# luigifreda/pyslam

Measured on AMD Instinct MI355X. Metric: RGB-D frames/sec fused (640x480, 5 mm voxel TSDF), higher is better.
Workload: dtype f32; 1 GPU; synthetic_640x480_5mm: synthetic 640x480 RGB-D @ 30 Hz stream, 5 mm TSDF (sdf_trunc 0.04 m, depth_trunc 4 m), 64 posed frames per step resident in HBM, Open3D ScalableTSDFVolume semantics; mode=multi-frame sweep (hv_tsdf_integrate_batch), units_allocated=31946, parity_pinned=False, clock_ramp_steps=60, full=False, build_digest=135281701958bda57bf956d25b5e2e59f6e6b8a8ce9266cc3e6c719ccc494ef5

## Files before the change

pyslam_amd/csrc/hv_tsdf.hip:

```cpp
#include <algorithm>
#include <array>
#include <cmath>
#include <cstring>
#include <numeric>

#include "hv_tsdf_device.h"

__global__ __launch_bounds__(256) void k_tsdf_multiplier_table(HvFrameParams P, float *__restrict__ out) {
    const int i = blockIdx.x * blockDim.x + threadIdx.x;
    if (i >= P.H * P.W) return;
    out[i] = hv_multiplier(P, i % P.W, i / P.W);
}


__global__ __launch_bounds__(256) void k_tsdf_prep_touch(HvTable table, int32_t *__restrict__ stamp,
                                                          int32_t *__restrict__ list, int parity,
                                                          const void *__restrict__ depth_raw,
                                                          const uint8_t *__restrict__ rgb,
                                                          uint2 *__restrict__ frame_px, HvFrameParams P,
                                                          int n_touch_blocks) {
    const int64_t npx = (int64_t)P.H * P.W;
    if ((int)blockIdx.x >= n_touch_blocks) {
        const int64_t i = (int64_t)((int)blockIdx.x - n_touch_blocks) * blockDim.x + threadIdx.x;
        if (i >= npx) return;
// ... 69 lines not shown

template <int ZB>
__device__ __forceinline__ void hv_tsdf_slabs(const HvFrameParams &P, const uint2 *__restrict__ frame_px, char *__restrict__ unit, int wordb,
                                              float (&pc)[4][3], float inc0, float inc1, float inc2) {
    float tv[ZB][4];
    uint32_t cv[ZB][4];
    unsigned mask = 0;
    bool near_plane = false;
#pragma unroll
    for (int c = 0; c < 4; ++c) {
        const float e = pc[c][2] + (float)ZB * inc2;
        near_plane |= (int)(fminf(pc[c][2], e) < 0x1p-10f) & (int)(fmaxf(pc[c][2], e) > -0x1p-10f);
    }
    if (P.tiled || __any(near_plane)) {
#pragma unroll
        for (int zz = 0; zz < ZB; ++zz) {
#pragma unroll
            for (int c = 0; c < 4; ++c) {
                if (hv_tsdf_eval_fast<true, false>(P, frame_px, nullptr, pc[c][0], pc[c][1], pc[c][2], tv[zz][c], cv[zz][c]))
                    mask |= 1u << (zz * 4 + c);
                pc[c][0] += inc0;
                pc[c][1] += inc1;
                pc[c][2] += inc2;
            }
        }
    } else {
#pragma unroll
        for (int zz = 0; zz < ZB; ++zz) {
#pragma unroll
            for (int c = 0; c < 4; ++c) {
                if (hv_tsdf_eval_fast<false, false>(P, frame_px, nullptr, pc[c][0], pc[c][1], pc[c][2], tv[zz][c], cv[zz][c]))
                    mask |= 1u << (zz * 4 + c);
                pc[c][0] += inc0;
                pc[c][1] += inc1;
                pc[c][2] += inc2;
            }
        }
    }
    float4 vt[ZB];
    uint4 vw[ZB], vr[ZB], vg[ZB], vb[ZB];
#pragma unroll
    for (int zz = 0; zz < ZB; ++zz) {
        if ((mask >> (zz * 4)) & 15u) {
            const int q = (wordb + zz * HV_TSDF_RR) >> 2;
            vt[zz] = ((const float4 *)(unit + 0 * HV_TSDF_PLANE_BYTES))[q];
            vw[zz] = ((const uint4 *)(unit + 1 * HV_TSDF_PLANE_BYTES))[q];
            vr[zz] = ((const uint4 *)(unit + 2 * HV_TSDF_PLANE_BYTES))[q];
            vg[zz] = ((const uint4 *)(unit + 3 * HV_TSDF_PLANE_BYTES))[q];
            vb[zz] = ((const uint4 *)(unit + 4 * HV_TSDF_PLANE_BYTES))[q];
        }
    }
#pragma unroll
    for (int zz = 0; zz < ZB; ++zz) {
        const unsigned m = (mask >> (zz * 4)) & 15u;
        if (m) {
            hv_tsdf_apply(m & 1u, tv[zz][0], cv[zz][0], vt[zz].x, vw[zz].x, vr[zz].x, vg[zz].x, vb[zz].x);
            hv_tsdf_apply(m & 2u, tv[zz][1], cv[zz][1], vt[zz].y, vw[zz].y, vr[zz].y, vg[zz].y, vb[zz].y);
            hv_tsdf_apply(m & 4u, tv[zz][2], cv[zz][2], vt[zz].z, vw[zz].z, vr[zz].z, vg[zz].z, vb[zz].z);
            hv_tsdf_apply(m & 8u, tv[zz][3], cv[zz][3], vt[zz].w, vw[zz].w, vr[zz].w, vg[zz].w, vb[zz].w);
            const int q = (wordb + zz * HV_TSDF_RR) >> 2;
            ((float4 *)(unit + 0 * HV_TSDF_PLANE_BYTES))[q] = vt[zz];
            ((uint4 *)(unit + 1 * HV_TSDF_PLANE_BYTES))[q] = vw[zz];
            ((uint4 *)(unit + 2 * HV_TSDF_PLANE_BYTES))[q] = vr[zz];
            ((uint4 *)(unit + 3 * HV_TSDF_PLANE_BYTES))[q] = vg[zz];
            ((uint4 *)(unit + 4 * HV_TSDF_PLANE_BYTES))[q] = vb[zz];
        }
    }
}

__global__ __launch_bounds__(256) void k_tsdf_integrate(HvTable table, const int32_t *__restrict__ list,
                                                         int parity, char *__restrict__ pool,
                                                         const uint2 *__restrict__ frame_px, HvFrameParams P,
                                                         HvStatus *status, int32_t status_seq) {
    int n_touched = table.counters[HV_CNT_TOUCH(parity)];
    if (n_touched > table.max_blocks) n_touched = table.max_blocks;
    if (blockIdx.x == 0 && threadIdx.x == 0) {
        table.counters[HV_CNT_TOUCH(parity ^ 1)] = 0;
        hv_publish_status(table, status, status_seq);
    }
    const int wave = threadIdx.x >> 6;
    const int lane = threadIdx.x & 63;
    const int x = lane >> 2;
    const int y0 = (lane & 3) << 2;
    const int z0 = wave * 4;
    const float inc0 = P.ext_scaled_col2[0], inc1 = P.ext_scaled_col2[1], inc2 = P.ext_scaled_col2[2];

    for (int t = blockIdx.x; t < n_touched; t += gridDim.x) {
        const int32_t slot = list[t];
        const int32_t idx = table.vals[slot];
        if (idx < 0) continue;
        int32_t ux, uy, uz;
        hv_unpack_key(table.keys[slot], ux, uy, uz);
        const double o0 = (double)ux * P.unit_length;
        const double o1 = (double)uy * P.unit_length;
        const double o2 = (double)uz * P.unit_length;
        const float p0 = (float)((double)(P.half_voxel_length_f + P.voxel_length_f * (float)x) + o0);
        const float p2 = (float)((double)P.half_voxel_length_f + o2);
        float pc[4][3];
#pragma unroll
        for (int c = 0; c < 4; ++c) {
            const float p1 = (float)((double)(P.half_voxel_length_f + P.voxel_length_f * (float)(y0 + c)) + o1);
#pragma unroll
            for (int r = 0; r < 3; ++r) {
                pc[c][r] = ((P.ext[r * 4 + 0] * p0 + P.ext[r * 4 + 1] * p1) + P.ext[r * 4 + 2] * p2) + P.ext[r * 4 + 3];
            }
        }
        for (int s = 0; s < z0; ++s) {
#pragma unroll
            for (int c = 0; c < 4; ++c) {
                pc[c][0] += inc0;
                pc[c][1] += inc1;
                pc[c][2] += inc2;
            }
        }
        char *unit = pool + (int64_t)idx * HV_TSDF_UNIT_BYTES;
        constexpr int ZB = 2;
#pragma unroll
        for (int zb = 0; zb < 4; zb += ZB) hv_tsdf_slabs<ZB>(P, frame_px, unit, hv_tsdf_word(x, y0, z0 + zb), pc, inc0, inc1, inc2);
    }
}

__device__ __forceinline__ void hv_touch_batch_patch(const HvTable &table, const HvFrameParams &P, const void *depth_f, const int patch,
                                                     HvTouchScratch &scratch, const int f, unsigned long long *__restrict__ frame_mask,
                                                     int32_t *__restrict__ stamp, int32_t *__restrict__ list, const int batch_stamp,
                                                     const int parity) {
    const unsigned long long fbit = 1ull << f;
    hv_touch_patch(table, P, depth_f, patch, scratch,
                   [&](unsigned long long key, int32_t ux, int32_t uy, int32_t uz) {
                       if (!hv_unit_hits_tile(P, ux, uy, uz)) return;
                       const int32_t slot = hv_table_insert(table, key);
                       if (slot < 0) return;
                       const unsigned long long seen = __hip_atomic_load(&frame_mask[slot], __ATOMIC_RELAXED, __HIP_MEMORY_SCOPE_AGENT);
                       const int32_t stamped = __hip_atomic_load(&stamp[slot], __ATOMIC_RELAXED, __HIP_MEMORY_SCOPE_AGENT);
                       if (!(seen & fbit)) atomicOr(&frame_mask[slot], fbit);
                       if (stamped != batch_stamp) {
                           const int32_t old = atomicExch(&stamp[slot], batch_stamp);
                           if (old != batch_stamp) {
                               const int32_t at = atomicAdd(&table.counters[HV_CNT_TOUCH(parity)], 1);
                               if (at < table.max_blocks) list[at] = slot;
                           }
                       }
                   });
}

__global__ __launch_bounds__(256) void k_tsdf_prep_touch_batch(HvTable table, int32_t *__restrict__ stamp,
                                                                unsigned long long *__restrict__ frame_mask,
                                                                int32_t *__restrict__ list, int batch_stamp,
                                                                const char *__restrict__ depth_raw, int64_t depth_stride,
                                                                const uint8_t *__restrict__ rgb,
                                                                uint2 *__restrict__ frame_px,
                                                                const HvFrameParams *__restrict__ Ps, int n_prep_blocks,
                                                                int n_touch_blocks, int n_frames, int parity,
                                                                const float *__restrict__ mult12) {
    int f, bx;
    const bool touch_role = (int)blockIdx.x < n_touch_blocks * n_frames;
    if (touch_role) {
        f = (int)blockIdx.x / n_touch_blocks;
        bx = (int)blockIdx.x % n_touch_blocks;
    } else {
        const int b = (int)blockIdx.x - n_touch_blocks * n_frames;
        f = b / n_prep_blocks;
        bx = b % n_prep_blocks;
    }
    const HvFrameParams &P = Ps[f];
    const int64_t npx = (int64_t)P.H * P.W;
    const void *depth_f = depth_raw + (int64_t)f * depth_stride;
    const uint8_t *rgb_f = rgb + (int64_t)f * npx * 3;
    if (!touch_role) {
        hv_pack_px4(P, f, ((int64_t)bx * blockDim.x + threadIdx.x) * 4, depth_f, rgb_f, frame_px, mult12);
        return;
    }
    __shared__ HvTouchScratch scratch[4];
    const int patch = bx * 4 + (int)(threadIdx.x / HV_WAVE);
    if (patch < hv_touch_patches(P))
        hv_touch_batch_patch(table, P, depth_f, patch, scratch[threadIdx.x / HV_WAVE], f, frame_mask, stamp, list, batch_stamp, parity);
}

typedef float hv_f2 __attribute__((ext_vector_type(2)));

__device__ __forceinline__ hv_f2 hv_fma2(hv_f2 a, hv_f2 b, hv_f2 c) { return __builtin_elementwise_fma(a, b, c); }
__device__ __forceinline__ hv_f2 hv_splat(float x) { return hv_f2{x, x}; }

struct HvSweepFrameK {
    hv_f2 e04, e15, e26, e37;
    float e8, e11;
    hv_f2 e9_10, i01;
    float i2;
};
__device__ __forceinline__ HvSweepFrameK hv_sweep_frame_k(const HvFrameParams *__restrict__ Ps, int f) {
    const float *k = Ps[f].sweep_k;
    return HvSweepFrameK{hv_f2{k[0], k[1]}, hv_f2{k[2], k[3]}, hv_f2{k[4], k[5]}, hv_f2{k[6], k[7]}, k[8], k[9], hv_f2{k[10], k[11]}, hv_f2{k[12], k[13]}, k[14]};
}

static constexpr unsigned HV_SWEEP_XCD_GROUP = 2;
__device__ __forceinline__ int hv_sweep_items(const int n_units, const int parts) {
    constexpr int G = HV_SWEEP_XCD_GROUP;
    return (n_units + 8 * G - 1) / (8 * G) * 8 * G * parts;
}
__device__ __forceinline__ void hv_sweep_item(const unsigned item, const unsigned parts, int &t, int &part) {
    constexpr unsigned G = HV_SWEEP_XCD_GROUP;
    const unsigned xcd = item & 7u, j = item >> 3;
    const unsigned g = j / (G * parts), within = j % (G * parts);
    t = (int)((g * 8 + xcd) * G + within / parts);
    part = (int)(within % parts);
}

static constexpr int HV_WAIT_VMCNT0 = 0x0f70;
struct HvPlaneWords {
    float vt;
    uint32_t vw, r, g, b;
};
template <int ZH, int ZB, bool TW, typename Updated, typename Finish>
__device__ __forceinline__ void hv_sweep_epilogue(char *__restrict__ unit, const int wordb, Updated updated, Finish finish) {
    constexpr int NP = ZH / ZB;
    static_assert(ZH % ZB == 0, "whole passes");
    auto load = [&](const int p, HvPlaneWords (&w)[ZB]) __attribute__((always_inline)) {
#pragma unroll
        for (int k = 0; k < ZB; ++k) {
            const int z = p * ZB + k;
            if (updated(z)) {
                const int q = wordb + z * HV_TSDF_RR;
                if (TW) {
                    w[k].vt = ((const float *)(unit + 0 * HV_TSDF_PLANE_BYTES))[q];
                    w[k].vw = ((const uint32_t *)(unit + 1 * HV_TSDF_PLANE_BYTES))[q];
                }
                w[k].r = ((const uint32_t *)(unit + 2 * HV_TSDF_PLANE_BYTES))[q];
                w[k].g = ((const uint32_t *)(unit + 3 * HV_TSDF_PLANE_BYTES))[q];
                w[k].b = ((const uint32_t *)(unit + 4 * HV_TSDF_PLANE_BYTES))[q];
            }
        }
    };
    auto store = [&](const int p, const HvPlaneWords (&w)[ZB]) __attribute__((always_inline)) {
#pragma unroll
        for (int k = 0; k < ZB; ++k) {
            const int z = p * ZB + k;
            if (updated(z)) {
                const int q = wordb + z * HV_TSDF_RR;
                HvPlaneWords o = w[k];
                finish(z, o);
                ((float *)(unit + 0 * HV_TSDF_PLANE_BYTES))[q] = o.vt;
                ((uint32_t *)(unit + 1 * HV_TSDF_PLANE_BYTES))[q] = o.vw;
                ((uint32_t *)(unit + 2 * HV_TSDF_PLANE_BYTES))[q] = o.r;
                ((uint32_t *)(unit + 3 * HV_TSDF_PLANE_BYTES))[q] = o.g;
                ((uint32_t *)(unit + 4 * HV_TSDF_PLANE_BYTES))[q] = o.b;
            }
        }
    };
#pragma unroll
    for (int p = 0; p < NP; ++p) {
        HvPlaneWords w[ZB];
        load(p, w);
        __builtin_amdgcn_sched_barrier(0);
        __builtin_amdgcn_s_waitcnt(HV_WAIT_VMCNT0);
        store(p, w);
        __builtin_amdgcn_sched_barrier(0);
    }
}

static constexpr int HV_SWEEP_ZH = 4;
static constexpr int HV_SWEEP_SPLIT = 8;
static constexpr int HV_SWEEP_WAVES = 64 / HV_SWEEP_ZH / HV_SWEEP_SPLIT;
static constexpr int HV_SWEEP_WPE = 4;
static_assert(HV_SWEEP_ZH % 2 == 0, "voxels are folded in pairs");

struct HvSweepGather {
    uint2 rec[HV_SWEEP_ZH];
    float mm[HV_SWEEP_ZH], zk[HV_SWEEP_ZH];
    bool ok[HV_SWEEP_ZH];
};

__global__ __launch_bounds__(64 * HV_SWEEP_WAVES, HV_SWEEP_WPE) void k_tsdf_sweep(
    HvTable table, const int32_t *__restrict__ list, const unsigned long long *__restrict__ frame_mask,
    char *__restrict__ pool, const uint2 *__restrict__ frame_px, const HvFrameParams *__restrict__ Ps, int n_frames,
    int general, const float *__restrict__ mult, int parity) {
    constexpr int ZH = HV_SWEEP_ZH, SPLIT = HV_SWEEP_SPLIT, WAVES = HV_SWEEP_WAVES;
    int n_units = table.counters[HV_CNT_TOUCH(parity)];
    if (n_units > table.max_blocks) n_units = table.max_blocks;
    const int wave = __builtin_amdgcn_readfirstlane(threadIdx.x >> 6);
    const int lane = threadIdx.x & 63;
    const HvFrameParams &P0 = Ps[0];
    const float vl = P0.voxel_length_f, hl = P0.half_voxel_length_f;
    const double unit_length = P0.unit_length;
    const bool tiled = P0.tiled != 0;
    const int npx = P0.H * P0.W;
    const hv_f2 F = {P0.fx, P0.fy}, C = {P0.cx, P0.cy};
    const uint32_t lo = __float_as_uint(0.0001f);
    const uint32_t wlim = __float_as_uint(P0.safe_width_f) - lo, hlim = __float_as_uint(P0.safe_height_f) - lo;
    const uint32_t W24 = (uint32_t)P0.W;
    const float ntrunc = -P0.sdf_trunc_f, tinv = P0.sdf_trunc_inv_f;
    const __amdgpu_buffer_rsrc_t rs_m = __builtin_amdgcn_make_buffer_rsrc((void *)mult, 0, npx * 4, 0x00020000);
    const int n_items = hv_sweep_items(n_units, SPLIT);
    for (int item = blockIdx.x; item < n_items; item += gridDim.x) {
        int t, part;
        hv_sweep_item(item, SPLIT, t, part);
        if (t >= n_units) continue;
        const int task = part * WAVES + wave;
        const int cg = task & 3;
        const int z0 = (task >> 2) * ZH;
        const int x = cg * 4 + (lane >> 4);
        const int y = lane & 15;
        const int32_t slot = list[t];
        const int32_t idx = table.vals[slot];
        unsigned long long mask = frame_mask[slot];
        if (idx < 0 || mask == 0ull) continue;
        int32_t ux, uy, uz;
        hv_unpack_key(table.keys[slot], ux, uy, uz);
        const double o0 = (double)ux * unit_length, o1 = (double)uy * unit_length, o2 = (double)uz * unit_length;
        bool near = false;
        if (lane < n_frames && ((mask >> lane) & 1ull)) {
            const HvFrameParams &Pl = Ps[lane];
            const float bx = (float)((double)(hl + vl * (float)(cg * 4)) + o0), by = (float)((double)hl + o1),
                        bz = (float)((double)(hl + vl * (float)z0) + o2);
            const float zmin = (Pl.ext[8] * bx + Pl.ext[9] * by + Pl.ext[10] * bz + Pl.ext[11]) + fminf(Pl.ext[8] * (3.0f * vl), 0.f) +
                               fminf(Pl.ext[9] * (15.0f * vl), 0.f) + fminf(Pl.ext[10] * ((float)(ZH - 1) * vl), 0.f);
            near = !(zmin > 0.03f);
        }
        const bool near_any = __any(near);
        char *unit = pool + (int64_t)idx * HV_TSDF_UNIT_BYTES;
        const int wordb = z0 * HV_TSDF_RR + cg * 64 + lane;
        float vt[ZH];
        uint32_t vw[ZH];
#pragma unroll
        for (int zz = 0; zz < ZH; ++zz) {
            const int q = wordb + zz * HV_TSDF_RR;
            vt[zz] = ((const float *)(unit + 0 * HV_TSDF_PLANE_BYTES))[q];
// ... 552 lines not shown
    for (int attempt = 0;; ++attempt) {
        tsdf_next_frame(v, P, parity);
        if (attempt > 0) HV_HIP(hipMemsetAsync(&v->table.counters[HV_CNT_TOUCH0], 0, HV_CNT_TOUCH_SPAN_BYTES, v->stream));
        rc = tsdf_launch_touch(v, v->stream, P, parity, d_depth, d_rgb);
        if (rc != HV_OK) return rc;
        if (!checked) break;
        rc = hv_claims_fit(v);
        if (rc == HV_OK) break;
        if (rc != HV_RETRY_CLAIM || attempt >= 8) return rc == HV_RETRY_CLAIM ? HV_ERR_CAPACITY : rc;
        make_frame_params(v, H, W, intr, T_cw, depth_scale, depth_trunc, depth_dtype, &P);
    }
    return tsdf_launch_integrate(v, P, parity);
}

int check_tsdf_args(hv_volume *v, const void *depth, const uint8_t *rgb, int H, int W,
                           const double *intr, const double *T_cw, int frames) {
    HV_REQUIRE(v != nullptr, HV_ERR_INVALID, "hv_tsdf_integrate: null volume");
    HV_REQUIRE(v->cfg.mode == HV_MODE_TSDF, HV_ERR_MODE, "hv_tsdf_integrate: volume is not in TSDF mode");
    HV_REQUIRE(depth != nullptr && rgb != nullptr && intr != nullptr && T_cw != nullptr, HV_ERR_INVALID,
               "[ScalableTSDFVolume::Integrate] Unsupported image format.");
    HV_REQUIRE(H > 0 && W > 0 && frames > 0, HV_ERR_INVALID, "hv_tsdf_integrate: empty image");
    HV_REQUIRE((int64_t)H * W <= v->cfg.max_points, HV_ERR_CAPACITY,
               "hv_tsdf_integrate: image %dx%d exceeds max_points=%lld", W, H, (long long)v->cfg.max_points);
    return HV_OK;
}

extern "C" {

int hv_tsdf_integrate(hv_volume *v, const void *depth, int32_t depth_dtype, const uint8_t *rgb,
                      int32_t height, int32_t width, const double *intr, const double *T_cw,
                      double depth_scale, double depth_trunc, int32_t loc) {
    int rc = check_tsdf_args(v, depth, rgb, height, width, intr, T_cw, 1);
    if (rc != HV_OK) return rc;
    HV_HIP(hipSetDevice(v->device));
    const size_t npx = (size_t)height * width;
    const void *d_depth = nullptr;
    const uint8_t *d_rgb = nullptr;
    rc = hv_stage_frame(v, depth, depth_dtype, rgb, npx, loc, &d_depth, &d_rgb);
    if (rc != HV_OK) return rc;
    return tsdf_integrate_one(v, d_depth, depth_dtype, d_rgb, height, width, intr, T_cw,
                              depth_scale, depth_trunc);
}

}

size_t tsdf_batch_scratch(size_t rec_bytes, size_t npx, int B, size_t *params_offset) {
    const size_t px_bytes = rec_bytes * npx * (size_t)B;
    *params_offset = (px_bytes + 255) & ~(size_t)255;
    return px_bytes + 256 + sizeof(HvFrameParams) * (size_t)B;
}

int tsdf_integrate_batch_impl(hv_volume *v, const void *depth, const void *const *depth_ptrs, int32_t depth_dtype,
                                     const uint8_t *rgb, const void *const *rgb_ptrs, int32_t n_frames, int32_t height,
                                     int32_t width, const double *intr, const double *T_cw, double depth_scale,
                                     double depth_trunc, int32_t loc) {
    int rc = HV_OK;
    HV_HIP(hipSetDevice(v->device));
    const size_t npx = (size_t)height * width;
    const size_t dsz = depth_dtype == HV_DEPTH_U16 ? 2 : 4;
    const void *d_depth = nullptr, *d_rgb = nullptr;
    int host_set = -1;
    if (loc == HV_HOST) {
        rc = hv_stage_frames(v, depth_ptrs, depth, npx * dsz, rgb_ptrs, rgb, npx * 3, n_frames, &d_depth, &d_rgb, &host_set);
        if (rc != HV_OK) return rc;
    } else {
        d_depth = depth;
        d_rgb = rgb;
    }
    if (n_frames == 1) {
        if (host_set >= 0) HV_HIP(hipStreamWaitEvent(v->stream, v->hs_dev_ready[host_set], 0));
        rc = tsdf_integrate_one(v, d_depth, depth_dtype, (const uint8_t *)d_rgb, height, width, intr, T_cw, depth_scale, depth_trunc);
        if (rc != HV_OK) return rc;
        if (host_set >= 0) return hv_stage_frames_consumed(v, host_set, v->stream);
        return HV_OK;
    }
    const bool pipeline_on = !(getenv("HV_TSDF_PIPELINE") && atoi(getenv("HV_TSDF_PIPELINE")) == 0);
    const int sweep_form = getenv("HV_TSDF_SWEEP") && atoi(getenv("HV_TSDF_SWEEP")) == 2 ? 2 : 4;
    const bool rec12 = sweep_form == 4;
    const size_t rec_bytes = rec12 ? 12 : 8;
    const int general = getenv("HV_TSDF_BATCH_GENERAL") ? atoi(getenv("HV_TSDF_BATCH_GENERAL")) : 0;
    const int zs = getenv("HV_TSDF_SWEEP_ZS") ? atoi(getenv("HV_TSDF_SWEEP_ZS")) : (v->owner_world >= 4 ? 2 : 1);
    const int sweep_grid = 65536;
    bool chain_ok = v->pipe_armed && v->pipe_version == v->content_version;
    v->content_version += 1;
    const int BMAX = HV_BATCH_MAX;
    for (int f0 = 0; f0 < n_frames; f0 += BMAX) {
        const int B = std::min(BMAX, n_frames - f0);
        bool checked = false;
        const int64_t max_before = v->cfg.max_blocks;
        rc = hv_capacity_gate(v, &checked);
        if (rc != HV_OK) return rc;
        if (v->cfg.max_blocks != max_before) chain_ok = false;
        const bool overlap = pipeline_on && chain_ok && !checked;
        if (v->stream_aux == nullptr) {
            HV_HIP(hipStreamCreateWithFlags(&v->stream_aux, hipStreamNonBlocking));
            HV_HIP(hipEventCreateWithFlags(&v->ev_prep, hipEventDisableTiming));
            HV_HIP(hipEventCreateWithFlags(&v->ev_presweep, hipEventDisableTiming));
        }
        hipStream_t ps = overlap ? v->stream_aux : v->stream;
        bool overlap_this = overlap;
        const int parity = v->batch_parity & 1;
        v->batch_parity = parity ^ 1;
        int32_t *d_list = v->touched_list + (size_t)parity * (size_t)v->cfg.max_blocks;
        unsigned long long *d_mask_rw = (unsigned long long *)v->touched_mask + (size_t)parity * (size_t)v->table_capacity;
        if (overlap) HV_HIP(hipStreamWaitEvent(v->stream_aux, v->ev_presweep, 0));
        if (host_set >= 0) HV_HIP(hipStreamWaitEvent(ps, v->hs_dev_ready[host_set], 0));
        const int ri = v->params_idx;
        v->params_idx = (ri + 1) & 3;
        if (v->pinned_params[ri] == nullptr) {
            HV_HIP(hipHostMalloc(&v->pinned_params[ri], sizeof(HvFrameParams) * BMAX));
            HV_HIP(hipEventCreateWithFlags(&v->params_ev[ri], hipEventDisableTiming));
        } else {
            HV_HIP(hipEventSynchronize(v->params_ev[ri]));
        }
        HvFrameParams *params = (HvFrameParams *)v->pinned_params[ri];
        for (int f = 0; f < B; ++f) {
            make_frame_params(v, height, width, intr, T_cw + 16 * (size_t)(f0 + f), depth_scale, depth_trunc, depth_dtype,
                              &params[f]);
            v->frame_counter += 1;
            params[f].frame_id = v->frame_counter;
        }
        int batch_stamp = v->frame_counter;
        v->last_touch_parity = parity;
        {
            const float *before = v->mult_table;
            const int mw = v->mult_W, mh = v->mult_H;
            float key_before[4];
            memcpy(key_before, v->mult_key, sizeof(key_before));
            rc = tsdf_multiplier_table(v, params[0]);
            if (rc != HV_OK) return rc;
            if (before != v->mult_table || mw != v->mult_W || mh != v->mult_H || memcmp(key_before, v->mult_key, sizeof(key_before)) != 0) {
                if (ps != v->stream) HV_HIP(hipStreamSynchronize(v->stream_aux));
                ps = v->stream;
                overlap_this = false;
                if (host_set >= 0) HV_HIP(hipStreamWaitEvent(ps, v->hs_dev_ready[host_set], 0));
            }
        }
        const float *d_mult = v->mult_table;
        size_t params_off = 0;
        const size_t want = tsdf_batch_scratch(rec_bytes, npx, B, &params_off);
        void **bb = parity ? &v->batch_buf2 : &v->batch_buf;
        size_t *bb_bytes = parity ? &v->batch_buf2_bytes : &v->batch_buf_bytes;
        if (*bb_bytes < want && v->stream_aux) HV_HIP(hipStreamSynchronize(v->stream_aux));
        rc = hv_ensure_buffer(v, bb, bb_bytes, want);
        if (rc != HV_OK) return rc;
        uint2 *d_px = (uint2 *)*bb;
        HvFrameParams *d_params = (HvFrameParams *)((char *)*bb + params_off);
        {
            const int n16 = (int)((sizeof(HvFrameParams) * (size_t)B + 15) / 16);
            hipLaunchKernelGGL(k_upload_words, dim3(1), dim3(256), 0, ps, (const uint4 *)params, (uint4 *)d_params, n16);
        }
        HV_HIP(hipEventRecord(v->params_ev[ri], ps));
        const int n_prep_blocks = (int)((npx + 1023) / 1024);
        const int n_touch_blocks = (hv_touch_patches(width, height, v->cfg.depth_sampling_stride) + 3) / 4;
        const void *c_depth = (const char *)d_depth + npx * dsz * (size_t)f0;
        const uint8_t *c_rgb = (const uint8_t *)d_rgb + npx * 3 * (size_t)f0;
        rc = tsdf_rectify(v, ps, &c_depth, depth_dtype, &c_rgb, B, height, width);
        if (rc != HV_OK) return rc;
        for (int attempt = 0;; ++attempt) {
            if (!v->touch_counters_clean) HV_HIP(hipMemsetAsync(&v->table.counters[HV_CNT_TOUCH0], 0, HV_CNT_TOUCH_SPAN_BYTES, v->stream));
            v->touch_counters_clean = true;
            hipLaunchKernelGGL(k_tsdf_prep_touch_batch, dim3((n_prep_blocks + n_touch_blocks) * B), dim3(256), 0, ps,
                               v->table, v->touched_stamp, d_mask_rw, d_list, batch_stamp,
                               (const char *)c_depth, (int64_t)(npx * dsz), c_rgb, d_px, (const HvFrameParams *)d_params, n_prep_blocks, n_touch_blocks, B, parity,
                               rec12 ? d_mult : (const float *)nullptr);
            if (!checked) break;
            rc = hv_claims_fit(v);
            if (rc == HV_OK) break;
            if (rc != HV_RETRY_CLAIM || attempt >= 8) return rc == HV_RETRY_CLAIM ? HV_ERR_CAPACITY : rc;
            v->frame_counter += 1;
            batch_stamp = v->frame_counter;
            v->touch_counters_clean = false;
            d_list = v->touched_list + (size_t)parity * (size_t)v->cfg.max_blocks;
            d_mask_rw = (unsigned long long *)v->touched_mask + (size_t)parity * (size_t)v->table_capacity;
        }
        HV_HIP(hipEventRecord(v->ev_presweep, v->stream));
        if (overlap_this) {
            HV_HIP(hipEventRecord(v->ev_prep, v->stream_aux));
            HV_HIP(hipStreamWaitEvent(v->stream, v->ev_prep, 0));
        }
        chain_ok = true;
        hv_profile_begin(v);
        const unsigned long long *d_mask = d_mask_rw;
        if (sweep_form == 2)
            hipLaunchKernelGGL(k_tsdf_sweep, dim3(sweep_grid), dim3(64 * HV_SWEEP_WAVES), 0, v->stream, v->table, (const int32_t *)d_list, d_mask,
                               (char *)v->pool, (const uint2 *)d_px, (const HvFrameParams *)d_params, B, general, d_mult, parity);
        else if (zs == 2)
            hipLaunchKernelGGL(k_tsdf_sweep_column<2>, dim3(sweep_grid), dim3(64), 0, v->stream, v->table, (const int32_t *)d_list, d_mask,
                               (char *)v->pool, (const uint2 *)d_px, (const HvFrameParams *)d_params, B, general, d_mult, parity);
        else
            hipLaunchKernelGGL(k_tsdf_sweep_column<1>, dim3(sweep_grid), dim3(64), 0, v->stream, v->table, (const int32_t *)d_list, d_mask,
                               (char *)v->pool, (const uint2 *)d_px, (const HvFrameParams *)d_params, B, general, d_mult, parity);
        hv_profile_end(v, B);
        hipLaunchKernelGGL(k_tsdf_batch_finish, dim3(1), dim3(1024), 0, v->stream, v->table, (const int32_t *)d_list, d_mask_rw, parity, v->d_status,
                           hv_next_status_seq(v));
        HV_HIP(hipGetLastError());
    }
    v->pipe_armed = true;
    v->pipe_version = v->content_version;
    if (host_set >= 0) return hv_stage_frames_consumed(v, host_set, v->stream);
    return HV_OK;
}

extern "C" {

int hv_tsdf_integrate_batch(hv_volume *v, const void *depth, int32_t depth_dtype, const uint8_t *rgb,
                            int32_t n_frames, int32_t height, int32_t width, const double *intr,
                            const double *T_cw, double depth_scale, double depth_trunc, int32_t loc) {
    int rc = check_tsdf_args(v, depth, rgb, height, width, intr, T_cw, n_frames);
    if (rc != HV_OK) return rc;
    return tsdf_integrate_batch_impl(v, depth, nullptr, depth_dtype, rgb, nullptr, n_frames, height, width, intr, T_cw, depth_scale,
                                     depth_trunc, loc);
}

int hv_tsdf_integrate_frames(hv_volume *v, const void *const *depth_frames, int32_t depth_dtype, const uint8_t *const *rgb_frames,
                             int32_t n_frames, int32_t height, int32_t width, const double *intr, const double *T_cw,
                             double depth_scale, double depth_trunc) {
    HV_REQUIRE(depth_frames != nullptr && rgb_frames != nullptr && n_frames >= 1, HV_ERR_INVALID, "hv_tsdf_integrate_frames: null argument");
    for (int f = 0; f < n_frames; ++f)
        HV_REQUIRE(depth_frames[f] != nullptr && rgb_frames[f] != nullptr, HV_ERR_INVALID, "hv_tsdf_integrate_frames: null frame %d", f);
    int rc = check_tsdf_args(v, depth_frames[0], rgb_frames[0], height, width, intr, T_cw, n_frames);
    if (rc != HV_OK) return rc;
    return tsdf_integrate_batch_impl(v, nullptr, depth_frames, depth_dtype, nullptr, (const void *const *)rgb_frames, n_frames, height,
                                     width, intr, T_cw, depth_scale, depth_trunc, HV_HOST);
}

int hv_tsdf_set_tile(hv_volume *v, int32_t u0, int32_t v0, int32_t u1, int32_t v1) {
    HV_REQUIRE(v != nullptr, HV_ERR_INVALID, "hv_tsdf_set_tile: null volume");
    HV_REQUIRE(v->cfg.mode == HV_MODE_TSDF, HV_ERR_MODE, "hv_tsdf_set_tile: volume is not in TSDF mode");
    HV_REQUIRE((u0 == 0 && v0 == 0 && u1 == 0 && v1 == 0) || (u0 >= 0 && v0 >= 0 && u1 > u0 && v1 > v0), HV_ERR_INVALID,
               "hv_tsdf_set_tile: empty tile");
    v->tile[0] = u0;
    v->tile[1] = v0;
    v->tile[2] = u1;
    v->tile[3] = v1;
    return HV_OK;
}

int hv_tsdf_set_color_order(hv_volume *v, int32_t bgr) {
    HV_REQUIRE(v != nullptr, HV_ERR_INVALID, "hv_tsdf_set_color_order: null volume");
    HV_REQUIRE(v->cfg.mode == HV_MODE_TSDF, HV_ERR_MODE, "hv_tsdf_set_color_order: volume is not in TSDF mode");
    v->color_bgr = bgr ? 1 : 0;
    return HV_OK;
}

int hv_tsdf_set_owner(hv_volume *v, int32_t rank, int32_t world_size) {
    HV_REQUIRE(v != nullptr, HV_ERR_INVALID, "hv_tsdf_set_owner: null volume");
    HV_REQUIRE(v->cfg.mode == HV_MODE_TSDF, HV_ERR_MODE, "hv_tsdf_set_owner: volume is not in TSDF mode");
    HV_REQUIRE(world_size >= 1 && rank >= 0 && rank < world_size, HV_ERR_INVALID, "hv_tsdf_set_owner: bad rank/world");
    v->owner_rank = rank;
    v->owner_world = world_size;
    return HV_OK;
}

int hv_tsdf_dump(hv_volume *v, int32_t *keys, float *tsdf, float *weight, double *color, int64_t *n_units) {
    HV_REQUIRE(v != nullptr && n_units != nullptr, HV_ERR_INVALID, "hv_tsdf_dump: null argument");
    HV_REQUIRE(v->cfg.mode == HV_MODE_TSDF, HV_ERR_MODE, "hv_tsdf_dump: volume is not in TSDF mode");
    int64_t nb = 0;
    int rc = hv_num_blocks(v, &nb);
    if (rc != HV_OK) return rc;
    *n_units = nb;
    if (nb == 0 || (keys == nullptr && tsdf == nullptr && weight == nullptr && color == nullptr)) return HV_OK;
    std::vector<int32_t> order, xyz;
    rc = hv_tsdf_key_order(v, nb, order, &xyz);
    if (rc != HV_OK) return rc;
    std::vector<char> unit((size_t)HV_TSDF_UNIT_BYTES);
    for (int64_t o = 0; o < nb; ++o) {
        const int64_t i = order[o];
        if (keys) memcpy(keys + o * 3, &xyz[o * 3], 12);
        if (!(tsdf || weight || color)) continue;
        HV_HIP(hipMemcpy(unit.data(), (char *)v->pool + i * unit.size(), unit.size(), hipMemcpyDeviceToHost));
        const float *pt = (const float *)unit.data();
        const uint32_t *pw = (const uint32_t *)(unit.data() + HV_TSDF_PLANE_BYTES);
        const uint32_t *pr = (const uint32_t *)(unit.data() + 2 * HV_TSDF_PLANE_BYTES);
        const uint32_t *pg = (const uint32_t *)(unit.data() + 3 * HV_TSDF_PLANE_BYTES);
        const uint32_t *pb = (const uint32_t *)(unit.data() + 4 * HV_TSDF_PLANE_BYTES);
        for (int x = 0; x < HV_TSDF_R; ++x)
            for (int y = 0; y < HV_TSDF_R; ++y)
                for (int z = 0; z < HV_TSDF_R; ++z) {
                    const int src = hv_tsdf_word(x, y, z);
                    const int64_t dst = o * HV_TSDF_RRR + (x * HV_TSDF_R + y) * HV_TSDF_R + z;
                    if (tsdf) tsdf[dst] = pt[src];
                    if (weight) weight[dst] = (float)pw[src];
                    if (color) {
                        const double w = (double)pw[src];
                        color[dst * 3 + 0] = w > 0 ? (double)pr[src] / w : 0.0;
                        color[dst * 3 + 1] = w > 0 ? (double)pg[src] / w : 0.0;
                        color[dst * 3 + 2] = w > 0 ? (double)pb[src] / w : 0.0;
                    }
                }
    }
    return HV_OK;
}

int hv_tsdf_touched(hv_volume *v, int32_t *keys, int64_t cap, int64_t *n) {
    HV_REQUIRE(v != nullptr && n != nullptr, HV_ERR_INVALID, "hv_tsdf_touched: null argument");
    HV_REQUIRE(v->cfg.mode == HV_MODE_TSDF, HV_ERR_MODE, "hv_tsdf_touched: volume is not in TSDF mode");
    int rc = hv_read_counters(v);
    if (rc != HV_OK) return rc;
    int64_t nt = v->h_counters[HV_CNT_TOUCH(v->last_touch_parity)];
    if (nt > v->cfg.max_blocks) nt = v->cfg.max_blocks;
    *n = nt;
    if (keys == nullptr || nt == 0) return HV_OK;
    std::vector<int32_t> slots((size_t)nt);
    HV_HIP(hipMemcpy(slots.data(), v->touched_list, sizeof(int32_t) * nt, hipMemcpyDeviceToHost));
    std::vector<uint64_t> tkeys((size_t)v->table_capacity);
    HV_HIP(hipMemcpy(tkeys.data(), v->table.keys, sizeof(uint64_t) * v->table_capacity, hipMemcpyDeviceToHost));
    std::vector<std::array<int32_t, 3>> out((size_t)nt);
    for (int64_t i = 0; i < nt; ++i) hv_unpack_key(tkeys[slots[i]], out[i][0], out[i][1], out[i][2]);
    std::sort(out.begin(), out.end());
    const int64_t m = std::min(nt, cap);
    for (int64_t i = 0; i < m; ++i) memcpy(keys + i * 3, out[i].data(), 12);
    return HV_OK;
}

// ... 16 lines not shown
```

pyslam_amd/csrc/hv_tsdf_device.h:

```cpp
#pragma once
#include "hv_common.h"

static constexpr int HV_TOUCH_FAN = 8;
static constexpr uint32_t HV_REC_ONE = 1u << 24;

__device__ __forceinline__ uint32_t hv_colour_order(uint32_t c, int bgr) {
    return bgr ? __builtin_amdgcn_perm(0u, c, 0x03000102u) : c;
}

__device__ __forceinline__ float hv_multiplier(const HvFrameParams &P, int u, int v) {
    const float xx = ((float)u - P.cx) * P.ffl_inv_x;
    const float yy = ((float)v - P.cy) * P.ffl_inv_y;
    return sqrtf(xx * xx + yy * yy + 1.0f);
}

__device__ __forceinline__ float hv_convert_depth(const HvFrameParams &P, const void *depth_raw, int64_t i) {
    float p = P.depth_is_u16 ? (float)((const uint16_t *)depth_raw)[i] : ((const float *)depth_raw)[i];
    p = p / P.depth_scale_f;
    if ((double)p >= P.depth_trunc_d) p = 0.0f;
    return p;
}

__device__ inline bool hv_unit_hits_tile(const HvFrameParams &P, int32_t ux, int32_t uy, int32_t uz) {
    if (P.tile_u0 <= 0 && P.tile_v0 <= 0 && P.tile_u1 >= P.W && P.tile_v1 >= P.H) return true;
// ... 182 lines not shown
    float q = a * r;
    float rem = fmaf(-b, q, a);
    q = fmaf(rem, r, q);
    rem = fmaf(-b, q, a);
    return fmaf(rem, r, q);
}

__device__ __forceinline__ void hv_tsdf_apply(bool valid, float t, uint32_t c, float &tsdf, uint32_t &w, uint32_t &sr,
                                              uint32_t &sg, uint32_t &sb) {
    if (!valid) return;
    const float wf = (float)w;
    const float num = tsdf * wf + t;
    tsdf = (w < (1u << 24)) ? hv_div1(num, wf + 1.0f) : num / (wf + 1.0f);
    w += 1u;
    sr += c & 255u;
    sg += (c >> 8) & 255u;
    sb += (c >> 16) & 255u;
}


__device__ __forceinline__ float hv_sqrt_ge1(float x) {
    const float s = __builtin_amdgcn_sqrtf(x);
    const float sd = __uint_as_float(__float_as_uint(s) - 1u);
    const float su = __uint_as_float(__float_as_uint(s) + 1u);
    const float vp = fmaf(-sd, s, x);
    const float vs = fmaf(-su, s, x);
    float r = (vp <= 0.0f) ? sd : s;
    r = (vs > 0.0f) ? su : r;
    return r;
}

template <bool EXACT, bool MT, bool REC12 = false>
__device__ __forceinline__ bool hv_tsdf_eval_fast(const HvFrameParams &P, const uint2 *__restrict__ frame_px,
                                                  const float *__restrict__ mult, float pc0, float pc1, float pc2,
                                                  float &t, uint32_t &rgb) {
    const float a0 = pc0 * P.fx, a1 = pc1 * P.fy;
    float q0, q1;
    hv_div2(a0, a1, pc2, q0, q1);
    if (EXACT) {
        const bool tiny = !(pc2 >= 0x1p-20f);
        const float e0 = a0 / pc2, e1 = a1 / pc2;
        q0 = tiny ? e0 : q0;
        q1 = tiny ? e1 : q1;
    }
    const float u_f = q0 + P.cx + 0.5f;
    const float v_f = q1 + P.cy + 0.5f;
    const uint32_t lo = __float_as_uint(0.0001f);
    const bool in_u = (__float_as_uint(u_f) - lo) < (__float_as_uint(P.safe_width_f) - lo);
    const bool in_v = (__float_as_uint(v_f) - lo) < (__float_as_uint(P.safe_height_f) - lo);
    bool ok = (int)(pc2 > 0.0f) & (int)in_u & (int)in_v;
    const int u = (int)u_f;
    const int v = (int)v_f;
    if (EXACT && P.tiled) {
        const bool in_tile_u = (int)(u >= P.tile_u0) & (int)(u < P.tile_u1);
        const bool in_tile_v = (int)(v >= P.tile_v0) & (int)(v < P.tile_v1);
        ok = (int)ok & (int)in_tile_u & (int)in_tile_v;
    }
    const uint32_t off = ok ? (uint32_t)v * (uint32_t)P.W + (uint32_t)u : 0u;
    uint2 rec;
    float m;
    if (REC12) {
        const uint32_t *r3 = (const uint32_t *)frame_px + (size_t)off * 3;
        rec = make_uint2(r3[0], r3[1]);
        m = __uint_as_float(r3[2]);
    } else {
        rec = frame_px[off];
    }
    const float d = __uint_as_float(rec.x);
    if (REC12) {
    } else if (MT) {
        m = mult[off];
    } else {
        const float xx = ((float)u - P.cx) * P.ffl_inv_x;
        const float yy = ((float)v - P.cy) * P.ffl_inv_y;
        m = hv_sqrt_ge1(xx * xx + yy * yy + 1.0f);
    }
    const float sdf = (d - pc2) * m;
    ok = (int)ok & (int)(d > 0.0f) & (int)(sdf > -P.sdf_trunc_f);
    t = fminf(sdf * P.sdf_trunc_inv_f, 1.0f);
    rgb = rec.y;
    return ok;
}

__device__ __forceinline__ void hv_tsdf_apply_fast(bool ok, float t, uint32_t rgb, float &tsdf, float &wf, uint32_t &sr,
                                                   uint32_t &sg, uint32_t &sb) {
    const float wf1 = wf + 1.0f;
    const float nt = hv_div1(tsdf * wf + t, wf1);
    tsdf = ok ? nt : tsdf;
    wf = ok ? wf1 : wf;
    const uint32_t c = ok ? rgb : 0u;
    sr += c & 255u;
    sg += (c >> 8) & 255u;
    sb += (c >> 16) & 255u;
}

__device__ __forceinline__ void hv_pack_px4(const HvFrameParams &P, const int f, const int64_t i0, const void *depth_f,
                                            const uint8_t *rgb_f, uint2 *__restrict__ frame_px, const float *__restrict__ mult12) {
    const int64_t npx = (int64_t)P.H * P.W;
    if (i0 >= npx) return;
    if (P.tiled && (P.W & 3) == 0) {
        const int u = (int)(i0 % P.W), v = (int)(i0 / P.W);
        if (u + 3 < P.tile_u0 - 4 || u >= P.tile_u1 + 4 || v < P.tile_v0 - 4 || v >= P.tile_v1 + 4) return;
    }
    uint2 *dst = frame_px + (int64_t)f * npx + i0;
    uint32_t *dst12 = (uint32_t *)frame_px + ((int64_t)f * npx + i0) * 3;
    if (i0 + 4 <= npx && (npx & 3) == 0) {
        const uint32_t *c4 = (const uint32_t *)(rgb_f + i0 * 3);
        const uint32_t w0 = c4[0], w1 = c4[1], w2 = c4[2];
        const uint32_t col[4] = {hv_colour_order(w0 & 0xffffffu, P.bgr) | HV_REC_ONE,
                                 hv_colour_order((w0 >> 24) | ((w1 & 0xffffu) << 8), P.bgr) | HV_REC_ONE,
                                 hv_colour_order((w1 >> 16) | ((w2 & 0xffu) << 16), P.bgr) | HV_REC_ONE,
                                 hv_colour_order(w2 >> 8, P.bgr) | HV_REC_ONE};
        float d[4];
        if (P.depth_is_u16) {
            const uint2 raw = *(const uint2 *)((const uint16_t *)depth_f + i0);
            d[0] = (float)(raw.x & 0xffffu); d[1] = (float)(raw.x >> 16);
            d[2] = (float)(raw.y & 0xffffu); d[3] = (float)(raw.y >> 16);
        } else {
            const float4 raw = *(const float4 *)((const float *)depth_f + i0);
            d[0] = raw.x; d[1] = raw.y; d[2] = raw.z; d[3] = raw.w;
        }
#pragma unroll
        for (int k = 0; k < 4; ++k) {
            d[k] = d[k] / P.depth_scale_f;
            if ((double)d[k] >= P.depth_trunc_d) d[k] = 0.0f;
        }
        if (mult12 != nullptr) {
            const float4 m4 = *(const float4 *)(mult12 + i0);
            ((uint4 *)dst12)[0] = make_uint4(__float_as_uint(d[0]), col[0], __float_as_uint(m4.x), __float_as_uint(d[1]));
            ((uint4 *)dst12)[1] = make_uint4(col[1], __float_as_uint(m4.y), __float_as_uint(d[2]), col[2]);
            ((uint4 *)dst12)[2] = make_uint4(__float_as_uint(m4.z), __float_as_uint(d[3]), col[3], __float_as_uint(m4.w));
        } else {
            ((uint4 *)dst)[0] = make_uint4(__float_as_uint(d[0]), col[0], __float_as_uint(d[1]), col[1]);
            ((uint4 *)dst)[1] = make_uint4(__float_as_uint(d[2]), col[2], __float_as_uint(d[3]), col[3]);
        }
    } else {
        for (int64_t i = i0; i < npx && i < i0 + 4; ++i) {
            const uint8_t *c = rgb_f + i * 3;
            uint2 rec;
            rec.x = __float_as_uint(hv_convert_depth(P, depth_f, i));
            rec.y = hv_colour_order((uint32_t)c[0] | ((uint32_t)c[1] << 8) | ((uint32_t)c[2] << 16), P.bgr) | HV_REC_ONE;
            if (mult12 != nullptr) {
                uint32_t *r3 = (uint32_t *)frame_px + ((int64_t)f * npx + i) * 3;
                r3[0] = rec.x;
                r3[1] = rec.y;
                r3[2] = __float_as_uint(mult12[i]);
            } else {
                frame_px[(int64_t)f * npx + i] = rec;
            }
        }
    }
}

static constexpr int HV_BATCH_MAX = 64;
int make_frame_params(hv_volume *v, int H, int W, const double *intr, const double *T_cw, double depth_scale, double depth_trunc,
                      int depth_dtype, HvFrameParams *P);
int tsdf_multiplier_table(hv_volume *v, const HvFrameParams &P);
int tsdf_rectify(hv_volume *v, hipStream_t s, const void **depth, int depth_dtype, const uint8_t **rgb, int B, int H, int W);
int check_tsdf_args(hv_volume *v, const void *depth, const uint8_t *rgb, int H, int W, const double *intr, const double *T_cw,
                    int frames);
size_t tsdf_batch_scratch(size_t rec_bytes, size_t npx, int B, size_t *params_offset);
int tsdf_integrate_batch_impl(hv_volume *v, const void *depth, const void *const *depth_ptrs, int32_t depth_dtype, const uint8_t *rgb,
                              const void *const *rgb_ptrs, int32_t n_frames, int32_t height, int32_t width, const double *intr,
                              const double *T_cw, double depth_scale, double depth_trunc, int32_t loc);
```

Before: 65330 frames/s.

## Pack two frames per prep thread with wave-staged coalesced 12-byte record stores

Prep blocks in the batched prep/touch kernel now each pack two frames, reusing one multiplier-table load across both. The stores are restaged through LDS within a wave so the 12-byte pixel records go out as contiguous coalesced uint4 writes. Pixels outside a tiled region (plus a margin) are skipped, and a templated fast path handles the u16 and f32 depth formats. The aim is to cut scattered store traffic and the redundant multiplier loads in the pre-sweep pack, at the cost of fewer prep blocks, a larger code path, and a reliance on scratch being large enough for staging.

Measured after the change: 66000 frames/s, median of 6. 1.0% higher.

```diff
diff --git a/pyslam_amd/csrc/hv_tsdf.hip b/pyslam_amd/csrc/hv_tsdf.hip
--- a/pyslam_amd/csrc/hv_tsdf.hip
+++ b/pyslam_amd/csrc/hv_tsdf.hip
@@ -245,25 +245,39 @@
                                                                 const HvFrameParams *__restrict__ Ps, int n_prep_blocks,
                                                                 int n_touch_blocks, int n_frames, int parity,
                                                                 const float *__restrict__ mult12) {
-    int f, bx;
-    const bool touch_role = (int)blockIdx.x < n_touch_blocks * n_frames;
-    if (touch_role) {
-        f = (int)blockIdx.x / n_touch_blocks;
-        bx = (int)blockIdx.x % n_touch_blocks;
-    } else {
+    __shared__ __attribute__((aligned(16))) HvTouchScratch scratch[4];
+    static_assert(sizeof(HvTouchScratch) >= HV_WAVE * 48, "a wave stages 64 x 4 records of 12 bytes");
+    if ((int)blockIdx.x >= n_touch_blocks * n_frames) {
         const int b = (int)blockIdx.x - n_touch_blocks * n_frames;
-        f = b / n_prep_blocks;
-        bx = b % n_prep_blocks;
-    }
+        const int f0 = (b / n_prep_blocks) * HV_PACK_FRAMES;
+        const int nf = min(HV_PACK_FRAMES, n_frames - f0);
+        const HvFrameParams &P = Ps[f0];
+        const int64_t npx = (int64_t)P.H * P.W;
+        const int64_t i0 = ((int64_t)(b % n_prep_blocks) * blockDim.x + threadIdx.x) * 4;
+        if (mult12 != nullptr && (npx & 3) == 0 && nf == HV_PACK_FRAMES && i0 < npx) {
+            if (P.tiled && (P.W & 3) == 0) {
+                const int u = (int)(i0 % P.W), v = (int)(i0 / P.W);
+                if (u + 3 < P.tile_u0 - 4 || u >= P.tile_u1 + 4 || v < P.tile_v0 - 4 || v >= P.tile_v1 + 4) return;
+            }
+            uint4 *stage = (uint4 *)&scratch[threadIdx.x / HV_WAVE];
+            const bool whole_wave = __ballot(1) == ~0ull;
+            if (P.depth_is_u16) {
+                if (whole_wave) hv_pack_px4_frames<true, true>(P, f0, i0, depth_raw, depth_stride, rgb, frame_px, mult12, stage);
+                else hv_pack_px4_frames<true, false>(P, f0, i0, depth_raw, depth_stride, rgb, frame_px, mult12, nullptr);
+            } else {
+                if (whole_wave) hv_pack_px4_frames<false, true>(P, f0, i0, depth_raw, depth_stride, rgb, frame_px, mult12, stage);
+                else hv_pack_px4_frames<false, false>(P, f0, i0, depth_raw, depth_stride, rgb, frame_px, mult12, nullptr);
+            }
+            return;
+        }
+        for (int k = 0; k < nf; ++k)
+            hv_pack_px4(P, f0 + k, i0, depth_raw + (int64_t)(f0 + k) * depth_stride, rgb + (int64_t)(f0 + k) * npx * 3, frame_px, mult12);
+        return;
+    }
+    const int f = (int)blockIdx.x / n_touch_blocks;
+    const int bx = (int)blockIdx.x % n_touch_blocks;
     const HvFrameParams &P = Ps[f];
-    const int64_t npx = (int64_t)P.H * P.W;
     const void *depth_f = depth_raw + (int64_t)f * depth_stride;
-    const uint8_t *rgb_f = rgb + (int64_t)f * npx * 3;
-    if (!touch_role) {
-        hv_pack_px4(P, f, ((int64_t)bx * blockDim.x + threadIdx.x) * 4, depth_f, rgb_f, frame_px, mult12);
-        return;
-    }
-    __shared__ HvTouchScratch scratch[4];
     const int patch = bx * 4 + (int)(threadIdx.x / HV_WAVE);
     if (patch < hv_touch_patches(P))
         hv_touch_batch_patch(table, P, depth_f, patch, scratch[threadIdx.x / HV_WAVE], f, frame_mask, stamp, list, batch_stamp, parity);
@@ -1122,6 +1136,7 @@
         }
         HV_HIP(hipEventRecord(v->params_ev[ri], ps));
         const int n_prep_blocks = (int)((npx + 1023) / 1024);
+        const int n_pack_groups = (B + HV_PACK_FRAMES - 1) / HV_PACK_FRAMES;
         const int n_touch_blocks = (hv_touch_patches(width, height, v->cfg.depth_sampling_stride) + 3) / 4;
         const void *c_depth = (const char *)d_depth + npx * dsz * (size_t)f0;
         const uint8_t *c_rgb = (const uint8_t *)d_rgb + npx * 3 * (size_t)f0;
@@ -1130,7 +1145,7 @@
         for (int attempt = 0;; ++attempt) {
             if (!v->touch_counters_clean) HV_HIP(hipMemsetAsync(&v->table.counters[HV_CNT_TOUCH0], 0, HV_CNT_TOUCH_SPAN_BYTES, v->stream));
             v->touch_counters_clean = true;
-            hipLaunchKernelGGL(k_tsdf_prep_touch_batch, dim3((n_prep_blocks + n_touch_blocks) * B), dim3(256), 0, ps,
+            hipLaunchKernelGGL(k_tsdf_prep_touch_batch, dim3(n_touch_blocks * B + n_prep_blocks * n_pack_groups), dim3(256), 0, ps,
                                v->table, v->touched_stamp, d_mask_rw, d_list, batch_stamp,
                                (const char *)c_depth, (int64_t)(npx * dsz), c_rgb, d_px, (const HvFrameParams *)d_params, n_prep_blocks, n_touch_blocks, B, parity,
                                rec12 ? d_mult : (const float *)nullptr);
diff --git a/pyslam_amd/csrc/hv_tsdf_device.h b/pyslam_amd/csrc/hv_tsdf_device.h
--- a/pyslam_amd/csrc/hv_tsdf_device.h
+++ b/pyslam_amd/csrc/hv_tsdf_device.h
@@ -358,6 +358,69 @@
     }
 }
 
+static constexpr int HV_PACK_FRAMES = 2;
+
+template <bool U16, bool STAGE>
+__device__ __forceinline__ void hv_pack_px4_frames(const HvFrameParams &P, const int f0, const int64_t i0, const char *depth_raw,
+                                                   const int64_t depth_stride, const uint8_t *rgb, uint2 *__restrict__ frame_px,
+                                                   const float *__restrict__ mult12, uint4 *stage) {
+    constexpr int NF = HV_PACK_FRAMES;
+    const int64_t npx = (int64_t)P.H * P.W;
+    const float4 m = *(const float4 *)(mult12 + i0);
+    uint4 raw[NF];
+    uint32_t w[NF][3];
+#pragma unroll
+    for (int k = 0; k < NF; ++k) {
+        const char *depth_f = depth_raw + (int64_t)(f0 + k) * depth_stride;
+        if (U16) {
+            const uint2 r2 = *(const uint2 *)((const uint16_t *)depth_f + i0);
+            raw[k] = make_uint4(r2.x, r2.y, 0u, 0u);
+        } else {
+            raw[k] = *(const uint4 *)((const float *)depth_f + i0);
+        }
+        const uint32_t *c4 = (const uint32_t *)(rgb + ((int64_t)(f0 + k) * npx + i0) * 3);
+        w[k][0] = c4[0]; w[k][1] = c4[1]; w[k][2] = c4[2];
+    }
+#pragma unroll
+    for (int k = 0; k < NF; ++k) {
+        float d[4];
+        if (U16) {
+            d[0] = (float)(raw[k].x & 0xffffu); d[1] = (float)(raw[k].x >> 16);
+            d[2] = (float)(raw[k].y & 0xffffu); d[3] = (float)(raw[k].y >> 16);
+        } else {
+            d[0] = __uint_as_float(raw[k].x); d[1] = __uint_as_float(raw[k].y);
+            d[2] = __uint_as_float(raw[k].z); d[3] = __uint_as_float(raw[k].w);
+        }
+#pragma unroll
+        for (int j = 0; j < 4; ++j) {
+            d[j] = d[j] / P.depth_scale_f;
+            if ((double)d[j] >= P.depth_trunc_d) d[j] = 0.0f;
+        }
+        const uint32_t w0 = w[k][0], w1 = w[k][1], w2 = w[k][2];
+        const uint32_t col[4] = {hv_colour_order(w0 & 0xffffffu, P.bgr) | HV_REC_ONE,
+                                 hv_colour_order((w0 >> 24) | ((w1 & 0xffffu) << 8), P.bgr) | HV_REC_ONE,
+                                 hv_colour_order((w1 >> 16) | ((w2 & 0xffu) << 16), P.bgr) | HV_REC_ONE,
+                                 hv_colour_order(w2 >> 8, P.bgr) | HV_REC_ONE};
+        const uint4 r0 = make_uint4(__float_as_uint(d[0]), col[0], __float_as_uint(m.x), __float_as_uint(d[1]));
+        const uint4 r1 = make_uint4(col[1], __float_as_uint(m.y), __float_as_uint(d[2]), col[2]);
+        const uint4 r2 = make_uint4(__float_as_uint(m.z), __float_as_uint(d[3]), col[3], __float_as_uint(m.w));
+        uint4 *dst12 = (uint4 *)((uint32_t *)frame_px + ((int64_t)(f0 + k) * npx + i0) * 3);
+        if (STAGE) {
+            const int lane = hv_lane_id();
+            stage[lane * 3 + 0] = r0; stage[lane * 3 + 1] = r1; stage[lane * 3 + 2] = r2;
+            __builtin_amdgcn_fence(__ATOMIC_ACQ_REL, "wavefront");
+            __builtin_amdgcn_wave_barrier();
+            const uint4 a = stage[lane], b = stage[HV_WAVE + lane], c = stage[2 * HV_WAVE + lane];
+            __builtin_amdgcn_fence(__ATOMIC_ACQ_REL, "wavefront");
+            __builtin_amdgcn_wave_barrier();
+            uint4 *base = dst12 - lane * 3;
+            base[lane] = a; base[HV_WAVE + lane] = b; base[2 * HV_WAVE + lane] = c;
+        } else {
+            dst12[0] = r0; dst12[1] = r1; dst12[2] = r2;
+        }
+    }
+}
+
 static constexpr int HV_BATCH_MAX = 64;
 int make_frame_params(hv_volume *v, int H, int W, const double *intr, const double *T_cw, double depth_scale, double depth_trunc,
                       int depth_dtype, HvFrameParams *P);
```
